# Sudaraka88/LDWeaver

Measured on NVIDIA B200. Metric: weighted SNP-pair MI/sec, higher is better.
Workload: dtype int8 (tcgen05 kind::i8 with int32 accumulation of 28-bit fixed-point weights; fp32 MI epilogue, fp64 refinement of long-range links)

## Files before the change

### ldweaver_b200/csrc/mi_kernel.cuh

```cuda
#pragma once
#include "mi_types.h"
#include "umma.cuh"

namespace ldw {

constexpr int MI_EXP_WARPS = 6;
constexpr int MI_EXP_THREADS = 32 * MI_EXP_WARPS;
constexpr int MI_EPI_WARP0 = 8;
constexpr int MI_EPI_GROUPS = 4;
constexpr int MI_EPI_WARPS = 4 * MI_EPI_GROUPS;
constexpr int MI_EPI_THREADS = 32 * MI_EPI_WARPS;
constexpr int MI_THREADS = 32 * (MI_EPI_WARP0 + MI_EPI_WARPS);
#define LDW_STR2(x) #x
#define LDW_STR(x) LDW_STR2(x)
#define MI_REGS_CTRL 48
#define MI_REGS_EPI 96
static_assert(MI_EPI_WARP0 * 32 * MI_REGS_CTRL + MI_EPI_THREADS * MI_REGS_EPI <= MI_THREADS * ((65536 / MI_THREADS) & ~7), "register budget");
constexpr int MI_MAX_STAGES = 4;
constexpr uint32_t MI_ARR_BYTES = 128 * 128;
constexpr uint32_t MI_STAGE_REGION = 12 * MI_ARR_BYTES;
__host__ __device__ constexpr uint32_t mi_stage_need(int pa, int pb, int njlog2) {
  return (uint32_t)pa * MI_ARR_BYTES + 4u * (uint32_t)pb * (64u << njlog2);
}
__host__ __device__ constexpr int mi_stage_geo(int pa, int pb, int njlog2) {
  return mi_stage_need(pa, pb, njlog2) <= 3 * MI_ARR_BYTES ? 0 : mi_stage_need(pa, pb, njlog2) <= 4 * MI_ARR_BYTES ? 1 : 2;
}
__host__ __device__ constexpr int mi_geo_stages(int geo) { return 4 - geo; }
__host__ __device__ constexpr uint32_t mi_geo_bytes(int geo) { return geo == 0 ? 3 * MI_ARR_BYTES : geo == 1 ? 4 * MI_ARR_BYTES : 6 * MI_ARR_BYTES; }
constexpr uint32_t MI_JREC_BYTES = 128 * sizeof(Rec);
constexpr uint32_t MI_JDYN_BYTES = 128 * sizeof(ColDyn);
constexpr uint32_t MI_IREC_BYTES = 128 * sizeof(Rec);
constexpr uint32_t MI_IDYN_BYTES = 128 * sizeof(RowDyn);
constexpr uint32_t MI_BAR_BYTES = 512;
constexpr uint32_t MI_SMEM_BYTES = MI_STAGE_REGION + 2 * (MI_JREC_BYTES + MI_JDYN_BYTES) + MI_IREC_BYTES + MI_IDYN_BYTES + MI_BAR_BYTES + 1024;
static_assert(MI_SMEM_BYTES <= 232448, "shared memory budget (227 KB opt-in)");

__device__ __forceinline__ float lg2_fast(float x) {
  float y;
  asm("lg2.approx.ftz.f32 %0, %1;" : "=f"(y) : "f"(x));
  return y;
}
__device__ __forceinline__ uint32_t ld_volatile_u32(const uint32_t* p) {
  uint32_t v;
  asm volatile("ld.volatile.global.u32 %0, [%1];" : "=r"(v) : "l"(p));
  return v;
}

__host__ __device__ constexpr int mi_jc(int pa, int pb) {
  return (pa + 1) * (pb + 1) <= 4 ? 8 : (pa + 1) * (pb + 1) <= 9 ? 4 : (pa + 1) * (pb + 1) <= 12 ? 2 : 1;
}
__host__ __device__ constexpr int mi_njlog2(int pa, int pb) {
  return pa * pb == 1 ? 7 : pa * pb == 2 ? 6 : pa * pb <= 4 ? 5 : 4;
}

__device__ __noinline__ void lr_raise_threshold(const ScanParams& p, int lane) {
  constexpr int PER = MI_HIST_BINS / 32;
  uint32_t s = 0;
  for (int k = 0; k < PER; k++) s += ld_volatile_u32(p.hist + lane * PER + k);
  uint32_t suf = s;
#pragma unroll
  for (int o = 1; o < 32; o <<= 1) {
// ... 359 lines not shown
    case 10: epi_tile<3, 3, QC, RG>(p, c, rel); break;
    case 11: epi_tile<3, 4, QC, RG>(p, c, rel); break;
    case 12: epi_tile<4, 1, QC, RG>(p, c, rel); break;
    case 13: epi_tile<4, 2, QC, RG>(p, c, rel); break;
    case 14: epi_tile<4, 3, QC, RG>(p, c, rel); break;
    case 15: epi_tile<4, 4, QC, RG>(p, c, rel); break;
    default: break;
  }
}

template <bool DBG>
__global__ void __cluster_dims__(2, 1, 1) __launch_bounds__(MI_THREADS, 1)
mi_scan_kernel(const __grid_constant__ TmapSet tm, const __grid_constant__ ScanParams p) {
  extern __shared__ uint8_t smem_raw[];
  uint8_t* smem = reinterpret_cast<uint8_t*>((reinterpret_cast<uintptr_t>(smem_raw) + 1023) & ~(uintptr_t)1023);
  uint8_t* stage_base = smem;
  Rec* jrec = reinterpret_cast<Rec*>(smem + MI_STAGE_REGION);
  ColDyn* jdyn = reinterpret_cast<ColDyn*>(smem + MI_STAGE_REGION + 2 * MI_JREC_BYTES);
  Rec* irec = reinterpret_cast<Rec*>(smem + MI_STAGE_REGION + 2 * (MI_JREC_BYTES + MI_JDYN_BYTES));
  RowDyn* idyn = reinterpret_cast<RowDyn*>(smem + MI_STAGE_REGION + 2 * (MI_JREC_BYTES + MI_JDYN_BYTES) + MI_IREC_BYTES);
  uint64_t* bars = reinterpret_cast<uint64_t*>(smem + MI_STAGE_REGION + 2 * (MI_JREC_BYTES + MI_JDYN_BYTES) + MI_IREC_BYTES + MI_IDYN_BYTES);
  uint64_t* full = bars;
  uint64_t* empty = bars + 4;
  uint64_t* ready = bars + 8;
  uint64_t* tfull = bars + 12;
  uint64_t* tempty = bars + 14;
  uint64_t* jfull = bars + 16;
  uint64_t* jempty = bars + 18;
  uint64_t* drained = bars + 20;
  uint64_t* rfull = bars + 21;
  uint64_t* rempty = bars + 22;
  uint32_t* tmem_slot = reinterpret_cast<uint32_t*>(bars + 23);
  uint32_t* thdr = reinterpret_cast<uint32_t*>(bars + 24);

  const int warp = threadIdx.x >> 5, lane = threadIdx.x & 31;
  const uint32_t rank = cluster_ctarank();
  if (warp == 0 && lane == 0) {
    tma_prefetch_desc(&tm.a);
    for (int i = 0; i < MI_MAX_STAGES; i++) {
      mbar_init(&full[i], 1); mbar_init(&empty[i], 1); mbar_init(&ready[i], 2 * MI_EXP_WARPS);
    }
    mbar_init(drained, 1);
    mbar_init(rfull, 1); mbar_init(rempty, MI_EPI_WARPS);
    for (int i = 0; i < 2; i++) {
      mbar_init(&tfull[i], 1); mbar_init(&tempty[i], 2 * MI_EPI_WARPS);
      mbar_init(&jfull[i], 1); mbar_init(&jempty[i], MI_EPI_WARPS);
    }
    fence_barrier_init();
  }
  if (warp == 2) tmem_alloc_pair(tmem_slot, 512);
  tc_fence_before();
  cluster_sync_all();
  tc_fence_after();
  const uint32_t tmem_base = *tmem_slot;
  const int tile0 = (int)(blockIdx.x >> 1), tstep = (int)(gridDim.x >> 1);

  if (warp < MI_EPI_WARP0) {
  asm volatile("setmaxnreg.dec.sync.aligned.u32 " LDW_STR(MI_REGS_CTRL) ";");
  if (warp == 0) {
    int st = 0; uint32_t phb = 0; int geo = -1; uint32_t dph = 0;
    int it = 0, rit = 0;
    long long w_jempty = 0, w_empty = 0, t_begin = DBG ? clock64() : 0;
    for (int t = tile0; t < p.n_tiles; t += tstep, it++) {
      const TileDesc td = p.tiles[t];
      const int PA = td.PA, PB = td.PB, NJ = 1 << td.njlog2, NJh = NJ >> 1;
      const int njidx = 7 - td.njlog2;
      const int g = mi_stage_geo(PA, PB, td.njlog2);
      const int nst = mi_geo_stages(g);
      const uint32_t sbytes = mi_geo_bytes(g);
      if (g != geo) {
        if (geo >= 0) { mbar_wait(drained, dph, 12); dph ^= 1; }
        geo = g; st = 0;
      }
      {
        const uint32_t stage_tx = (uint32_t)PA * MI_ARR_BYTES + (uint32_t)(PB * NJh * 128);
        const int a_row = td.a_row0 + (int)rank * 128, b_row = td.b_row0 + (int)rank * NJh;
        for (int kb = 0; kb < p.nkb; kb++) {
          timed_wait<DBG>(&empty[st], ((phb >> st) & 1) ^ 1, 11, w_empty);
          if (elect_one()) {
            uint8_t* sb = stage_base + st * sbytes;
            mbar_arrive_expect_tx(&full[st], stage_tx);
            for (int a = 0; a < PA; a++)
              tma_load_2d(sb + a * MI_ARR_BYTES, &tm.a, &full[st], kb * 128, a_row + a * td.a_pstride);
            uint8_t* sbB = sb + PA * MI_ARR_BYTES;
            for (int b = 0; b < PB; b++)
              tma_load_2d(sbB + b * NJh * 128, &tm.b[njidx], &full[st], kb * 128, b_row + b * td.b_pstride);
          }
          __syncwarp();
          phb ^= 1u << st;
          if (++st == nst) st = 0;
        }
      }
      const int jb = it & 1;
      timed_wait<DBG>(&jempty[jb], ((it >> 1) & 1) ^ 1, 10, w_jempty);
      if (elect_one()) {
        thdr[jb] = (uint32_t)PA | ((uint32_t)PB << 8) | ((uint32_t)td.njlog2 << 16) | ((uint32_t)(rank ? td.flags1 : td.flags) << 24);
        mbar_arrive_expect_tx(&jfull[jb], (uint32_t)NJ * (uint32_t)(sizeof(Rec) + sizeof(ColDyn)));
        bulk_load_1d(jrec + jb * 128, p.rec + (int64_t)(PA + 1 - 2) * p.rec_vstride + td.j_slot0, NJ * sizeof(Rec), &jfull[jb]);
        bulk_load_1d(jdyn + jb * 128, p.coldyn + td.j_dyn0, NJ * sizeof(ColDyn), &jfull[jb]);
      }
      __syncwarp();
      if (!((rank ? td.flags1 : td.flags) & TILE_NULL)) {
        timed_wait<DBG>(rempty, (uint32_t)(rit & 1) ^ 1, 13, w_jempty);
        if (elect_one()) {
          mbar_arrive_expect_tx(rfull, MI_IREC_BYTES + MI_IDYN_BYTES);
          bulk_load_1d(irec, p.rec + (int64_t)(PB + 1 - 2) * p.rec_vstride + td.i_slot0 + (int)rank * 128, MI_IREC_BYTES, rfull);
          bulk_load_1d(idyn, p.rowdyn + td.i_dyn0 + (int)rank * 128, MI_IDYN_BYTES, rfull);
        }
        __syncwarp();
        rit++;
      }
    }
    if (DBG && p.dbg && lane == 0) {
      p.dbg[blockIdx.x * 16 + 0] = (unsigned long long)(clock64() - t_begin);
      p.dbg[blockIdx.x * 16 + 1] = (unsigned long long)w_jempty;
      p.dbg[blockIdx.x * 16 + 2] = (unsigned long long)w_empty;
    }
  } else if (warp == 1) {
    if (rank == 0) {
    int st = 0; uint32_t phb = 0; int geo = -1; int as = 0; uint32_t aph = 0;
    long long w_tempty = 0, w_ready = 0, t_begin = DBG ? clock64() : 0;
    const uint32_t desc_hi = (uint32_t)(make_smem_desc_sw128(0) >> 32);
    for (int t = tile0; t < p.n_tiles; t += tstep) {
      const TileDesc td = p.tiles[t];
      const int PA = td.PA, PB = td.PB, NJ = 1 << td.njlog2;
      const int g = mi_stage_geo(PA, PB, td.njlog2);
      const int nst = mi_geo_stages(g);
      const uint32_t sbytes = mi_geo_bytes(g);
      if (g != geo) { geo = g; st = 0; }
      bool sw = false;
      if (t + tstep < p.n_tiles) {
        const TileDesc tn = p.tiles[t + tstep];
        sw = mi_stage_geo(tn.PA, tn.PB, tn.njlog2) != g;
      }
      const bool big = 2 * PA * PB * NJ > 256;
      const uint32_t ncols = (uint32_t)(2 * PB * NJ);
      const uint32_t idesc_u = make_idesc_u8(256, ncols);
      const uint32_t idesc_s = make_idesc_s8u8(256, ncols);
      uint32_t dbase;
      if (big) {
        for (int s2 = 0; s2 < 2; s2++) {
          timed_wait<DBG>(&tempty[as], aph ^ 1, 20, w_tempty);
          if (++as == 2) { as = 0; aph ^= 1; }
        }
        dbase = tmem_base;
      } else {
        timed_wait<DBG>(&tempty[as], aph ^ 1, 21, w_tempty);
        dbase = tmem_base + as * 256;
      }
      tc_fence_after();
      {
        const uint32_t boff = (uint32_t)PA * MI_ARR_BYTES;
        const uint32_t b2off = boff + (uint32_t)(PB * NJ * 128);
        for (int kb = 0; kb < p.nkb; kb++) {
          timed_wait<DBG>(&ready[st], (phb >> st) & 1, 22, w_ready);
          tc_fence_after();
          const uint32_t lo = ((smem_u32(stage_base + st * sbytes) & 0x3FFFFu) >> 4) | (1u << 16);
          if (elect_one()) {
            const uint64_t dBa = ((uint64_t)desc_hi << 32) | (lo + (boff >> 4));
            const uint64_t dBb = ((uint64_t)desc_hi << 32) | (lo + (b2off >> 4));
            const uint32_t acc0 = kb > 0 ? 1u : 0u;
            for (int a = 0; a < PA; a++) {
              const uint64_t dx = ((uint64_t)desc_hi << 32) | (lo + (uint32_t)((a * MI_ARR_BYTES) >> 4));
              const uint32_t dHL = dbase + (uint32_t)(a * 2 * PB * NJ);
              umma_i8_pair(dHL, dx, dBa, idesc_u, acc0);
              umma_i8_pair(dHL, dx, dBb, idesc_s, 1u);
#pragma unroll
              for (int kk = 1; kk < 4; kk++) {
                umma_i8_pair(dHL, dx + 2 * kk, dBa + 2 * kk, idesc_u, 1u);
                umma_i8_pair(dHL, dx + 2 * kk, dBb + 2 * kk, idesc_s, 1u);
              }
            }
            umma_commit_pair(&empty[st]);
          }
          __syncwarp();
          phb ^= 1u << st;
          if (++st == nst) st = 0;
        }
      }
      if (elect_one()) {
        if (sw) umma_commit_pair(drained);
        if (big) {
          umma_commit_pair(&tfull[0]);
          umma_commit_pair(&tfull[1]);
        } else {
          umma_commit_pair(&tfull[as]);
        }
      }
      __syncwarp();
      if (!big) {
        if (++as == 2) { as = 0; aph ^= 1; }
      }
    }
    if (DBG && p.dbg && lane == 0) {
      p.dbg[blockIdx.x * 16 + 3] = (unsigned long long)(clock64() - t_begin);
      p.dbg[blockIdx.x * 16 + 4] = (unsigned long long)w_tempty;
      p.dbg[blockIdx.x * 16 + 5] = (unsigned long long)w_ready;
    }
    }
  } else {
    const int h = (warp - 2) * 32 + lane;
    int st = 0; uint32_t phb = 0; int geo = -1;
    long long w_full = 0, t_begin = DBG ? clock64() : 0;
    for (int t = tile0; t < p.n_tiles; t += tstep) {
      const TileDesc td = p.tiles[t];
      const int PA = td.PA, PB = td.PB, NJh = (1 << td.njlog2) >> 1;
      const int brows = PB * NJh;
      const int g = mi_stage_geo(PA, PB, td.njlog2);
      const int nst = mi_geo_stages(g);
      const uint32_t sbytes = mi_geo_bytes(g);
      if (g != geo) { geo = g; st = 0; }
      for (int kb = 0; kb < p.nkb; kb++) {
        const int cl = h & 7;
        const uint8_t* dg = p.dig + (int64_t)kb * 128 + cl * 16;
        const uint4 g0 = __ldg(reinterpret_cast<const uint4*>(dg));
        const uint4 g1 = __ldg(reinterpret_cast<const uint4*>(dg + p.kpad));
        const uint4 g2 = __ldg(reinterpret_cast<const uint4*>(dg + 2 * p.kpad));
        const uint4 g3 = __ldg(reinterpret_cast<const uint4*>(dg + 3 * p.kpad));
        timed_wait<DBG>(&full[st], (phb >> st) & 1, 40, w_full);
        const uint32_t yb = smem_u32(stage_base + st * sbytes) + (uint32_t)PA * MI_ARR_BYTES;
        const uint32_t slot = (uint32_t)brows * 128u;
        for (int r = h >> 3; r < brows; r += MI_EXP_THREADS / 8) {
          const uint32_t addr = yb + (uint32_t)r * 128u + (uint32_t)((cl ^ (r & 7)) * 16);
          const uint4 y = lds128(addr);
          sts128(addr + slot, make_uint4(y.x & g1.x, y.y & g1.y, y.z & g1.z, y.w & g1.w));
          sts128(addr + 2 * slot, make_uint4(y.x & g2.x, y.y & g2.y, y.z & g2.z, y.w & g2.w));
          sts128(addr + 3 * slot, make_uint4(y.x & g3.x, y.y & g3.y, y.z & g3.z, y.w & g3.w));
          sts128(addr, make_uint4(y.x & g0.x, y.y & g0.y, y.z & g0.z, y.w & g0.w));
        }
        fence_proxy_async_smem();
        __syncwarp();
        if (lane == 0) mbar_arrive_cluster(&ready[st], 0);
        phb ^= 1u << st;
        if (++st == nst) st = 0;
      }
    }
    if (DBG && p.dbg && h == 0) {
      p.dbg[blockIdx.x * 16 + 12] = (unsigned long long)(clock64() - t_begin);
      p.dbg[blockIdx.x * 16 + 13] = (unsigned long long)w_full;
    }
  }
  } else {
    asm volatile("setmaxnreg.inc.sync.aligned.u32 " LDW_STR(MI_REGS_EPI) ";");
    EpiCtx c;
    c.q = warp & 3;
    c.cg = (warp - MI_EPI_WARP0) >> 2;
    c.lane = lane;
    c.rank = (int)rank;
    int as = 0; uint32_t aph = 0;
    int it = 0, rit = 0;
    long long w_jfull = 0, w_tfull = 0, t_begin = DBG ? clock64() : 0;
    c.irec_saddr = smem_u32(irec);
    c.idyn_saddr = smem_u32(idyn);
    c.rempty_saddr = smem_u32(rempty);
    c.scr_saddr = smem_u32(bars + 32) + (uint32_t)(warp - MI_EPI_WARP0) * 4u;
    for (int t = tile0; t < p.n_tiles; t += tstep, it++) {
      const int jb = it & 1;
      timed_wait<DBG>(&jfull[jb], (it >> 1) & 1, 30, w_jfull);
      uint32_t hdr;
      asm volatile("ld.shared.u32 %0, [%1];" : "=r"(hdr) : "r"(smem_u32(&thdr[jb])));
      const int tPA = (int)(hdr & 0xFF), tPB = (int)((hdr >> 8) & 0xFF);
      c.tflags = hdr >> 24;
      const int NJ = 1 << ((hdr >> 16) & 0xFF);
      const bool big = 2 * tPA * tPB * NJ > 256;
      if (!(c.tflags & TILE_NULL)) { timed_wait<DBG>(rfull, (uint32_t)(rit & 1), 34, w_jfull); rit++; }
      long long c1 = DBG ? clock64() : 0;
      c.jrec_saddr = smem_u32(jrec + jb * 128);
      c.jdyn_saddr = smem_u32(jdyn + jb * 128);
      if (big) {
        uint32_t ph0 = aph;
        mbar_wait(&tfull[as], ph0, 31);
        int as1 = as ^ 1;
        uint32_t ph1 = (as == 1) ? (aph ^ 1) : aph;
        mbar_wait(&tfull[as1], ph1, 32);
        c.tmem_base = tmem_base + ((uint32_t)(c.q * 32) << 16);
      } else {
        mbar_wait(&tfull[as], aph, 33);
        c.tmem_base = tmem_base + ((uint32_t)(c.q * 32) << 16) + as * 256;
      }
      if constexpr (DBG) w_tfull += clock64() - c1;
      tc_fence_after();
      bool released = false;
      auto release_acc = [&]() {
        tc_fence_before();
        __syncwarp();
        if (big) {
          if (lane == 0) { mbar_arrive_cluster(&tempty[0], 0); mbar_arrive_cluster(&tempty[1], 0); }
          aph ^= 1;
        } else {
// ... 31 lines not shown
```

### ldweaver_b200/csrc/mi_scan.cu

```cuda
#include <algorithm>
#include <chrono>
#include <cmath>
#include <cub/cub.cuh>
#include <vector>

#include "../../include/ldw.h"
#include "ctx.h"
#include "hdw.h"
#include "mi_aux.cuh"
#include "mi_kernel.cuh"
#include "mi_scan.h"

using namespace ldw;

namespace {

struct Group {
  int32_t slot0 = 0, nslots = 0, row0 = 0, count = 0;
};

struct DevLinks {
  DevBuf pos1, pos2, c1, c2, len, blk, mi;
  int ensure(int64_t m) {
    size_t b4 = (size_t)(m > 0 ? m : 1) * 4, b8 = (size_t)(m > 0 ? m : 1) * 8;
// ... 576 lines not shown
  memset(&sp, 0, sizeof(sp));
  sp.tiles = D.tiles.as<TileDesc>();
  sp.n_tiles = H.n_real_tiles;
  sp.rec = P->d_rec.as<Rec>();
  sp.rec_vstride = P->nslots;
  sp.rowdyn = D.rowdyn.as<RowDyn>();
  sp.coldyn = D.coldyn.as<ColDyn>();
  sp.nkb = (int32_t)(P->Kpad / 128);
  sp.nf = H.nf; sp.nt = H.nt;
  sp.diag = H.diag; sp.ragged = H.ragged;
  sp.qcorr = (!H.diag && !(cfg.flags & LDW_SCAN_IDEAL_Q)) ? 1 : 0;
  sp.sr_only = (cfg.flags & LDW_SCAN_SR_ONLY) ? 1 : 0;
  sp.dig = P->d_dig.as<uint8_t>();
  sp.kpad = P->Kpad;
  sp.rfl_arr = D.rfl.as<uint8_t>();
  sp.rtl_arr = D.rtl.as<uint8_t>();
  sp.sa = P->sa;
  sp.sb = P->sb;
  sp.kT = (float)(std::ldexp(1.0, (int)P->sb) / P->scale);
  sp.M = P->M;
  for (int a = 0; a < 4; a++)
    for (int b = 0; b < 4; b++) {
      double ri = a + 2, rj = b + 2;
      double den = P->neff + 0.5 * ri * rj;
      const float den_f = (float)den, rkT = 1.0f / sp.kT, rden = 1.0f / den_f;
      sp.scale[a][b] = (float)(M_LN2 / den) * sp.kT;
      sp.q0s[a][b] = (float)(0.25 * ri * rj / den) * rkT;
      sp.qod[a][b] = (float)(0.25 / den) * rkT;
      sp.rp_qc[a][b] = rden * rkT;
      sp.rp_plain[a][b] = den_f * sp.kT;
    }
}

int launch_scan(const ldw_mi_plan* P, const ScanParams& sp, cudaStream_t st, int reserve = 0) {
  if (sp.n_tiles <= 0) return 0;
  int grid = 2 * std::min<int>(sp.n_tiles, std::max(1, (P->ctx->num_sms - reserve) / 2));
  if (sp.dbg) mi_scan_kernel<true><<<grid, MI_THREADS, MI_SMEM_BYTES, st>>>(P->tm, sp);
  else mi_scan_kernel<false><<<grid, MI_THREADS, MI_SMEM_BYTES, st>>>(P->tm, sp);
  LDW_CUDA(cudaGetLastError());
  return 0;
}

RefineParams make_refine_params(const ldw_mi_plan* P, const BlockDev& D, const BlockHost& H, const ScanCfg& cfg) {
  RefineParams R;
  R.codes = P->codes_dev;
  R.S = P->S;
  R.w = P->d_w.as<double>();
  R.p64 = P->d_p64.as<double>();
  R.r = P->d_r.as<uint8_t>();
  R.mask = P->d_mask.as<uint8_t>();
  R.from_idx = D.from_idx.as<int32_t>();
  R.to_idx = D.to_idx.as<int32_t>();
  R.rfl_arr = D.rfl.as<uint8_t>();
  R.rtl_arr = D.rtl.as<uint8_t>();
  R.nf = H.nf; R.nt = H.nt;
  R.ideal_q = (cfg.flags & LDW_SCAN_IDEAL_Q) ? 1 : 0;
  R.neff = P->neff;
  return R;
}

int validate_scan(const ldw_mi_plan* P, const ScanCfg& cfg) {
  if (!(cfg.g > 0) || cfg.g != std::floor(cfg.g) || cfg.g > 9.0e15) return set_error(LDW_ERR_ARG, "genome length g=%g must be a positive integer", cfg.g);
  if (!(cfg.sr_dist >= 0)) return set_error(LDW_ERR_ARG, "sr_dist must be >= 0");
  if (!P->pos_sorted) return set_error(LDW_ERR_UNSUPPORTED, "POS must be non-decreasing (the short-range slot layout relies on it)");
  if (P->n > 0 && ((double)P->pos.back() - (double)P->pos.front()) >= cfg.g) return set_error(LDW_ERR_UNSUPPORTED, "POS span must be smaller than the genome length g");
  return 0;
}

}
// ... 57 lines not shown
int ldw_mi_block_dense(ldw_mi_plan* P, int64_t block_index, double* mi_out, int64_t* nf_out, int64_t* nt_out) {
  if (!P) return set_error(LDW_ERR_ARG, "null plan");
  LDW_TRY(ctx_bind(P->ctx));
  cudaStream_t st = P->ctx->stream;
  ScanWS* W = get_ws(P->ctx);
  int bf = 0, bt = 0;
  {
    int64_t k = block_index;
    bool found = false;
    for (int i = 0; i < P->nranges && !found; i++)
      for (int j = i; j < P->nranges; j++) {
        if (k == 0) { bf = i; bt = j; found = true; break; }
        k--;
      }
    if (!found) return set_error(LDW_ERR_ARG, "block index out of range");
  }
  ScanCfg cfg{1e15, 0.0, 0, 0, 0};
  cfg.dense = 1;
  BlockHost& H = W->hring[0];
  BlockDev& D = W->ring[0];
  int e = prepare_block(P, bf, bt, cfg, H);
  if (e > 1) return e;
  if (nf_out) *nf_out = H.nf;
  if (nt_out) *nt_out = H.nt;
  if (!mi_out) return 0;
  LDW_TRY(upload_block(st, D, H));
  size_t cells = (size_t)H.nf * H.nt;
  LDW_TRY(W->d_dense.ensure(cells * 4));
  LDW_CUDA(cudaMemsetAsync(W->d_dense.p, 0, cells * 4, st));
  ScanParams sp;
  fill_scan_params(P, D, H, cfg, sp);
  sp.dense = 1;
  sp.dense_out = W->d_dense.as<float>();
  LDW_TRY(launch_scan(P, sp, st));
  DevBuf d64;
  LDW_TRY(d64.alloc(cells * 8));
  f32_to_f64_kernel<<<(unsigned)((cells + 255) / 256), 256, 0, st>>>(W->d_dense.as<float>(), (int64_t)cells, d64.as<double>());
  LDW_CUDA(cudaMemcpyAsync(mi_out, d64.p, cells * 8, cudaMemcpyDeviceToHost, st));
  LDW_CUDA(cudaStreamSynchronize(st));
  return 0;
}

int ldw_mi_pairs_exact(ldw_mi_plan* P, int64_t block_index, const int32_t* from_local, const int32_t* to_local,
                       int64_t n_pairs, double* mi_out) {
  if (!P) return set_error(LDW_ERR_ARG, "null plan");
  LDW_TRY(ctx_bind(P->ctx));
  cudaStream_t st = P->ctx->stream;
  ScanWS* W = get_ws(P->ctx);
  int bf = 0, bt = 0;
  {
    int64_t k = block_index;
    bool found = false;
    for (int i = 0; i < P->nranges && !found; i++)
      for (int j = i; j < P->nranges; j++) {
        if (k == 0) { bf = i; bt = j; found = true; break; }
        k--;
      }
    if (!found) return set_error(LDW_ERR_ARG, "block index out of range");
  }
  if (n_pairs <= 0) return 0;
  ScanCfg cfg{1e15, 0.0, 0, 0, 0};
  BlockHost& H = W->hring[0];
  BlockDev& D = W->ring[0];
  int e = prepare_block(P, bf, bt, cfg, H);
  if (e != 0) return e == 1 ? set_error(LDW_ERR_ARG, "empty block") : e;
  for (int64_t k = 0; k < n_pairs; k++)
    if (from_local[k] < 0 || from_local[k] >= H.nf || to_local[k] < 0 || to_local[k] >= H.nt)
// ... 246 lines not shown
      first_rc = -1;
    } else {
      e = prepare_block(P, blocks[b].bf, blocks[b].bt, cfg, H);
    }
    if (e > 1) return e;
    LDW_TRY(upload_block(P->ctx->upload_stream, D, H));
    LDW_CUDA(cudaEventRecord(D.uploaded, P->ctx->upload_stream));
    LDW_CUDA(cudaStreamWaitEvent(st, D.uploaded, 0));
    host_prep_ms += std::chrono::duration<double, std::milli>(std::chrono::steady_clock::now() - hp0).count();
    D.used = true;
    ScanParams sp;
    fill_scan_params(P, D, H, cfg, sp);
    sp.sr_out = W->d_sr_f32.as<float>() + s.sr_base;
    if (dbg_block >= 0 && (int64_t)b == dbg_block) {
      LDW_TRY(W->d_dbg.ensure(4096 * 16 * 8));
      LDW_CUDA(cudaMemsetAsync(W->d_dbg.p, 0, 4096 * 16 * 8, st));
      sp.dbg = W->d_dbg.as<unsigned long long>();
    }
    const bool lr = !sr_only && s.n_lr > 0;
    const int emit_all = force_emit_all || s.emit_all;
    uint32_t cap = cap_override ? cap_override : s.cap;
    if (lr) {
      if (L.used) LDW_CUDA(cudaStreamWaitEvent(st, L.sel_done, 0));
      const int n_pilot = (int)H.tiles.size() - H.n_real_tiles;
      if (seq == 0 && use_chain && !emit_all && n_pilot > 0) {
        mi_block_begin_kernel<<<1, 256, 0, st>>>(d_count, L.hist.as<uint32_t>(), d_chain, 0);
        ScanParams pp = sp;
        pp.tiles = D.tiles.as<TileDesc>() + H.n_real_tiles;
        pp.n_tiles = n_pilot;
        pp.cand = L.cand.as<Cand>(); pp.cand_cap = cap; pp.cand_count = d_count; pp.tcand_bits = d_tcand;
        pp.hist = L.hist.as<uint32_t>(); pp.kprime = s.kprime; pp.delta = s.delta ? s.delta : 1; pp.overflow = d_overflow;
        pp.emit_all = 1;
        pp.dbg = nullptr;
        LDW_TRY(launch_scan(P, pp, st, 0));
        mi_pilot_seed_kernel<<<1, 1024, 0, st>>>(L.cand.as<Cand>(), d_count, cap, (unsigned long long)s.k_lo, (double)s.n_lr, d_chain);
        LDW_CUDA(cudaGetLastError());
        n_launches += 3;
      }
      if (force_seed >= 0.f && use_chain && !emit_all) {
        static_assert(sizeof(float) == 4, "float bits");
        LDW_CUDA(cudaMemcpyAsync(d_chain, &force_seed, 4, cudaMemcpyHostToDevice, st));
        LDW_CUDA(cudaStreamSynchronize(st));
      }
      mi_block_begin_kernel<<<1, 256, 0, st>>>(d_count, L.hist.as<uint32_t>(), d_chain, (use_chain && !emit_all) ? 1 : 0);
      LDW_CUDA(cudaGetLastError());
      n_launches++;
      sp.cand = L.cand.as<Cand>();
      sp.cand_cap = cap;
      sp.cand_count = d_count;
      sp.tcand_bits = d_tcand;
      sp.hist = L.hist.as<uint32_t>();
      sp.kprime = s.kprime;
      sp.delta = s.delta ? s.delta : 1;
      sp.overflow = d_overflow;
      sp.emit_all = emit_all;
    } else {
      sp.sr_only = 1;
    }
    if (sp.n_tiles > 0) {
      cudaEvent_t k0, k1;
      LDW_CUDA(cudaEventCreate(&k0));
      LDW_CUDA(cudaEventCreate(&k1));
      kev.push_back(k0);
      kev.push_back(k1);
      LDW_CUDA(cudaEventRecord(k0, st));
      LDW_TRY(launch_scan(P, sp, st, lr ? scan_reserve : 0));
      LDW_CUDA(cudaEventRecord(k1, st));
      n_launches++; n_scan_launches++;
      n_tiles += sp.n_tiles;
      for (int32_t ti = 0; ti < H.n_real_tiles; ti++) {
        const TileDesc& td = H.tiles[ti];
        exec_ops += 8.0 * 256.0 * (double)(td.PA * td.PB * (1 << td.njlog2)) * (double)P->Kpad;
        const int RA = td.PA + 1, RB = td.PB + 1;
        const int halves = ((td.flags & TILE_NULL) ? 0 : 1) + ((td.flags1 & TILE_NULL) ? 0 : 1);
        exec_mufu += halves * 128.0 * (double)(1 << td.njlog2) * (double)(RA * (RB + (sp.qcorr ? (RB + 1) / 2 : 0)));
      }
    }
    if (lr) {
      n_launches += 2;
      LDW_CUDA(cudaEventRecord(L.scan_done, st));
      LDW_CUDA(cudaStreamWaitEvent(sst, L.scan_done, 0));
      RefineParams R = make_refine_params(P, D, H, cfg);
      n_launches++;
      mi_presel_kernel<<<1, 1024, 0, sst>>>(L.cand.as<Cand>(), d_count, cap, d_tcand, emit_all, (unsigned long long)s.k_lo, (float)sel_margin,
                                           L.vcand.as<Cand>(), d_count + 5);
      LDW_CUDA(cudaGetLastError());
      mi_refine_list_kernel<<<P->ctx->num_sms * 4, 32 * REFINE_WARPS, 0, sst>>>(R, L.vcand.as<Cand>(), d_count + 5, L.mi64.as<double>());
      LDW_CUDA(cudaGetLastError());
      SelectParams q;
      memset(&q, 0, sizeof(q));
      q.cand = L.vcand.as<Cand>(); q.mi64 = L.mi64.as<double>(); q.vcount = d_count + 5; q.count = d_count; q.cap = cap;
      q.overflow = d_overflow; q.tcand_bits = d_tcand; q.emit_all = emit_all;
      q.k_lo = s.k_lo; q.k_hi = s.k_hi; q.h = s.h; q.interpolate = s.interp;
      q.tol_safe = sel_margin; q.tol_border = 1e-9;
      q.from_idx = D.from_idx.as<int32_t>(); q.to_idx = D.to_idx.as<int32_t>();
      q.nf = H.nf; q.nt = H.nt; q.diag = H.diag; q.block = (int32_t)blocks[b].index;
      q.kept_key = W->d_kept_key.as<uint64_t>(); q.kept_gi = W->d_kept_gi.as<int32_t>(); q.kept_gj = W->d_kept_gj.as<int32_t>();
      q.kept_mi = W->d_kept_mi.as<double>(); q.kept_count = W->d_kept_count.as<unsigned long long>(); q.kept_cap = kept_cap;
      q.kept_overflow = d_kept_overflow;
// ... 226 lines not shown
      double gaps = 0, gmax = 0;
      std::string detail;
      for (size_t k = 1; k + 1 < kev.size(); k += 2) {
        float ms = 0;
        cudaEventElapsedTime(&ms, kev[k], kev[k + 1]);
        gaps += ms;
        gmax = std::max<double>(gmax, ms);
        char b[32];
        snprintf(b, sizeof(b), " %.0f", 1e3 * ms);
        detail += b;
      }
      float first = 0, last = 0;
      cudaEventElapsedTime(&first, ev0, kev[0]);
      cudaEventElapsedTime(&last, kev[kev.size() - 1], ev1);
      fprintf(stderr, "ldw timing: gaps between scan kernels: sum %.3f ms, max %.3f ms; before first %.3f ms, after last %.3f ms; us:%s\n",
              gaps, gmax, first, last, detail.c_str());
    }
    stats_out->n_scan_launches = n_scan_launches;
    stats_out->n_launches = n_launches;
    stats_out->n_tiles = n_tiles;
    stats_out->exec_int8_ops = exec_ops;
    stats_out->t_host_prep_ms = host_prep_ms;
    stats_out->exec_mufu_ops = exec_mufu;
    {
      double em = 0;
      for (size_t b = 0; b < blocks.size(); b++)
        if (!sel[b].skip && sel[b].n_lr > 0 && !sr_only) em = std::max(em, (double)P->results[b].eps_obs);
      stats_out->eps_obs_max = em;
    }
  }
  if (dbg_block >= 0 && W->d_dbg.p) {
    std::vector<unsigned long long> h(4096 * 16);
    cudaMemcpy(h.data(), W->d_dbg.p, h.size() * 8, cudaMemcpyDeviceToHost);
    double s[16] = {0};
    int nb = 0;
    for (int c = 0; c < 4096; c++)
      if (h[c * 16 + 3]) { nb++; for (int k = 0; k < 16; k++) s[k] += (double)h[c * 16 + k]; }
    if (nb) {
      fprintf(stderr, "ldw dbg block %lld (%d CTAs, kilo-cycles avg): producer total %.0f wait_jempty %.0f wait_empty %.0f | "
              "mma total %.0f wait_tempty %.0f wait_ready %.0f | expander total %.0f wait_full %.0f | epi(first) total %.0f "
              "wait_jfull %.0f wait_tfull %.0f | epi(last) total %.0f wait_jfull %.0f wait_tfull %.0f\n", (long long)dbg_block, nb,
              s[0] / nb / 1e3, s[1] / nb / 1e3, s[2] / nb / 1e3, s[3] / nb / 1e3, s[4] / nb / 1e3, s[5] / nb / 1e3, s[12] / nb / 1e3,
              s[13] / nb / 1e3, s[6] / nb / 1e3, s[7] / nb / 1e3, s[8] / nb / 1e3, s[9] / nb / 1e3, s[10] / nb / 1e3, s[11] / nb / 1e3);
    }
  }
  kev_cleanup();
  cudaEventDestroy(ev0); cudaEventDestroy(ev1); cudaEventDestroy(ev2); cudaEventDestroy(ev3);
  lap("borderline + stats (host)");
  return 0;
}
```

### ldweaver_b200/csrc/mi_types.h

```cpp
#pragma once
#include <cuda.h>
#include <stdint.h>

namespace ldw {

struct __align__(16) Rec {
  uint32_t T[4];
  float rp[4];
  float q[4];
  uint32_t T4;
  float rp4;
  float q4;
  uint32_t pad;
};
static_assert(sizeof(Rec) == 64, "Rec must be 64 bytes");

struct RowDyn {
  int32_t il;
  float rtl;
};

struct __align__(16) ColDyn {
  int32_t jl;
  float rfl;
  int32_t a0, a1, b0, b1;
  uint32_t baseU, baseL;
};
static_assert(sizeof(ColDyn) == 32, "ColDyn must be 32 bytes");

enum : uint32_t { TILE_HAS_SR = 1u, TILE_NULL = 2u };

struct __align__(16) TileDesc {
  int32_t a_row0, a_pstride;
  int32_t b_row0, b_pstride;
  int32_t i_slot0, j_slot0;
  int32_t i_dyn0, j_dyn0;
  uint8_t PA, PB, njlog2, flags;
  uint8_t flags1, pad8[3];
  int32_t pad[2];
};
static_assert(sizeof(TileDesc) == 48, "TileDesc must be 48 bytes");

struct Cand {
  int32_t il, jl;
  float mi;
};

constexpr int MI_HIST_BINS = 4096;

struct ScanParams {
  const TileDesc* tiles;
  int32_t n_tiles;
  const Rec* rec;
  int64_t rec_vstride;
  const RowDyn* rowdyn;
  const ColDyn* coldyn;
  int32_t nkb;
  int32_t nf, nt;
  int32_t diag, ragged, qcorr, sr_only, dense, emit_all;
  const uint8_t* rfl_arr;
  const uint8_t* rtl_arr;
  float kT;
  uint32_t sa, sb;
  uint32_t M;
  float scale[4][4];
  float q0s[4][4];
  float qod[4][4];
  float rp_qc[4][4];
  float rp_plain[4][4];
  float* sr_out;
  float* dense_out;
  Cand* cand;
  uint32_t cand_cap;
  uint32_t* cand_count;
  uint32_t* tcand_bits;
  uint32_t* hist;
  uint32_t kprime, delta;
  uint32_t* overflow;
  const uint8_t* dig;
  int64_t kpad;
  unsigned long long* dbg;
};

struct TmapSet {
  CUtensorMap a;
  CUtensorMap b[4];
};

}
```

### ldweaver_b200/csrc/umma.cuh

```cuda
#pragma once
#include <cuda_runtime.h>
#include <stdint.h>
#include <stdio.h>

namespace ldw {

__device__ __forceinline__ uint32_t smem_u32(const void* p) { return (uint32_t)__cvta_generic_to_shared(p); }

__device__ __forceinline__ bool elect_one() {
  uint32_t pred;
  asm volatile(
      "{\n"
      ".reg .pred P;\n"
      "elect.sync _|P, 0xffffffff;\n"
      "selp.u32 %0, 1, 0, P;\n"
      "}\n"
      : "=r"(pred));
  return pred != 0;
}

__device__ __forceinline__ void mbar_init(uint64_t* bar, uint32_t count) {
  asm volatile("mbarrier.init.shared::cta.b64 [%0], %1;" ::"r"(smem_u32(bar)), "r"(count) : "memory");
}
__device__ __forceinline__ void fence_barrier_init() { asm volatile("fence.mbarrier_init.release.cluster;" ::: "memory"); }
__device__ __forceinline__ void fence_proxy_async_smem() { asm volatile("fence.proxy.async.shared::cta;" ::: "memory"); }
__device__ __forceinline__ void mbar_arrive_expect_tx(uint64_t* bar, uint32_t bytes) {
  asm volatile("mbarrier.arrive.expect_tx.shared::cta.b64 _, [%0], %1;" ::"r"(smem_u32(bar)), "r"(bytes) : "memory");
}
__device__ __forceinline__ void mbar_arrive(uint64_t* bar) {
  asm volatile("mbarrier.arrive.shared::cta.b64 _, [%0];" ::"r"(smem_u32(bar)) : "memory");
}
__device__ __forceinline__ bool mbar_try_wait(uint64_t* bar, uint32_t parity) {
  uint32_t ok;
  asm volatile(
      "{\n"
      ".reg .pred p;\n"
      "mbarrier.try_wait.parity.shared::cta.b64 p, [%1], %2, %3;\n"
      "selp.u32 %0, 1, 0, p;\n"
      "}\n"
      : "=r"(ok)
      : "r"(smem_u32(bar)), "r"(parity), "r"(0x989680u)
      : "memory");
  return ok != 0;
}
__device__ __forceinline__ uint64_t globaltimer_ns() {
  uint64_t t;
  asm volatile("mov.u64 %0, %%globaltimer;" : "=l"(t));
  return t;
}
#ifndef LDW_WAIT_TIMEOUT_NS
#define LDW_WAIT_TIMEOUT_NS 4000000000ull
#endif
__device__ __forceinline__ void mbar_wait(uint64_t* bar, uint32_t parity, int tag = 0) {
  if (mbar_try_wait(bar, parity)) return;
  uint32_t spins = 0;
  uint64_t t0 = 0;
  while (!mbar_try_wait(bar, parity)) {
    if ((++spins & 0x3FFu) == 0) {
      uint64_t now = globaltimer_ns();
      if (t0 == 0) t0 = now;
      if (now - t0 > LDW_WAIT_TIMEOUT_NS) {
        printf("ldw: mbarrier wait timeout tag=%d block=%d thread=%d parity=%u\n", tag, (int)blockIdx.x,
               (int)threadIdx.x, parity);
        __trap();
      }
    }
  }
}

__device__ __forceinline__ void mbar_arrive_cluster(uint64_t* bar, uint32_t rank) {
  uint32_t ra;
  asm volatile("mapa.shared::cluster.u32 %0, %1, %2;" : "=r"(ra) : "r"(smem_u32(bar)), "r"(rank));
  asm volatile("mbarrier.arrive.shared::cluster.b64 _, [%0];" ::"r"(ra) : "memory");
}
// ... 146 lines not shown
```

Before: 85.95 billion.

## Keep A rows resident in shared memory across runs of consecutive tiles

Persistent CTAs now process contiguous runs of tiles rather than a strided sequence. When a tile's A panels for all k-blocks fit in shared memory, they stay resident and are reused by following tiles with the same A row, so only B is streamed through a smaller ring; per-slot aempty barriers guard the reuse. The producer also issues the j-record and i-record bulk loads opportunistically inside the k-loop using test_wait, so it no longer blocks on them afterwards. This cuts redundant A TMA traffic, at the cost of fewer B stages, more complex barrier logic, and possible load imbalance from coarser tile runs.

```diff
diff --git a/ldweaver_b200/csrc/mi_kernel.cuh b/ldweaver_b200/csrc/mi_kernel.cuh
--- a/ldweaver_b200/csrc/mi_kernel.cuh
+++ b/ldweaver_b200/csrc/mi_kernel.cuh
@@ -27,6 +27,32 @@
 }
 __host__ __device__ constexpr int mi_geo_stages(int geo) { return 4 - geo; }
 __host__ __device__ constexpr uint32_t mi_geo_bytes(int geo) { return geo == 0 ? 3 * MI_ARR_BYTES : geo == 1 ? 4 * MI_ARR_BYTES : 6 * MI_ARR_BYTES; }
+constexpr int MI_MAX_ASLOTS = (int)(MI_STAGE_REGION / MI_ARR_BYTES);
+__host__ __device__ constexpr uint32_t mi_bstage_bytes(int pb, int njlog2) { return 4u * (uint32_t)pb * (64u << njlog2); }
+__host__ __device__ constexpr int mi_res_stages(int pa, int pb, int njlog2, int nkb) {
+  if (pa * nkb > MI_MAX_ASLOTS) return 0;
+  const uint32_t rest = MI_STAGE_REGION - (uint32_t)(pa * nkb) * MI_ARR_BYTES, b = mi_bstage_bytes(pb, njlog2);
+  return rest >= 4 * b ? 4 : rest >= 3 * b ? 3 : rest >= 2 * b ? 2 : 0;
+}
+struct MiGeo {
+  int id, nst;
+  uint32_t stride, bofs;
+  bool res;
+};
+__host__ __device__ inline MiGeo mi_geo(int pa, int pb, int njlog2, int nkb, bool stream_rows) {
+  const int nr = stream_rows ? 0 : mi_res_stages(pa, pb, njlog2, nkb);
+  MiGeo g;
+  if (nr) {
+    g.stride = mi_bstage_bytes(pb, njlog2);
+    g.id = 0x100 | (pa << 6) | (int)(g.stride >> 10);
+    g.nst = nr; g.bofs = (uint32_t)(pa * nkb) * MI_ARR_BYTES; g.res = true;
+  } else {
+    g.id = mi_stage_geo(pa, pb, njlog2);
+    g.nst = mi_geo_stages(g.id); g.stride = mi_geo_bytes(g.id); g.bofs = (uint32_t)pa * MI_ARR_BYTES; g.res = false;
+  }
+  return g;
+}
+__device__ __forceinline__ int mi_next_tile(int t, int R, int skip) { return (t + 1) % R == 0 ? t + 1 + skip : t + 1; }
 constexpr uint32_t MI_JREC_BYTES = 128 * sizeof(Rec);
 constexpr uint32_t MI_JDYN_BYTES = 128 * sizeof(ColDyn);
 constexpr uint32_t MI_IREC_BYTES = 128 * sizeof(Rec);
@@ -452,6 +478,8 @@
   uint64_t* rempty = bars + 22;
   uint32_t* tmem_slot = reinterpret_cast<uint32_t*>(bars + 23);
   uint32_t* thdr = reinterpret_cast<uint32_t*>(bars + 24);
+  uint64_t* aempty = bars + 40;
+  static_assert((40 + MI_MAX_ASLOTS) * 8 <= MI_BAR_BYTES, "barrier area");
 
   const int warp = threadIdx.x >> 5, lane = threadIdx.x & 31;
   const uint32_t rank = cluster_ctarank();
@@ -460,6 +488,7 @@
     for (int i = 0; i < MI_MAX_STAGES; i++) {
       mbar_init(&full[i], 1); mbar_init(&empty[i], 1); mbar_init(&ready[i], 2 * MI_EXP_WARPS);
     }
+    for (int i = 0; i < MI_MAX_ASLOTS; i++) mbar_init(&aempty[i], 1);
     mbar_init(drained, 1);
     mbar_init(rfull, 1); mbar_init(rempty, MI_EPI_WARPS);
     for (int i = 0; i < 2; i++) {
@@ -473,85 +502,99 @@
   cluster_sync_all();
   tc_fence_after();
   const uint32_t tmem_base = *tmem_slot;
-  const int tile0 = (int)(blockIdx.x >> 1), tstep = (int)(gridDim.x >> 1);
+  const int tile0 = (int)(blockIdx.x >> 1) * p.run_tiles;
+  const int tskip = (int)((gridDim.x >> 1) - 1) * p.run_tiles;
 
   if (warp < MI_EPI_WARP0) {
   asm volatile("setmaxnreg.dec.sync.aligned.u32 " LDW_STR(MI_REGS_CTRL) ";");
   if (warp == 0) {
     int st = 0; uint32_t phb = 0; int geo = -1; uint32_t dph = 0;
     int it = 0, rit = 0;
-    long long w_jempty = 0, w_empty = 0, t_begin = DBG ? clock64() : 0;
-    for (int t = tile0; t < p.n_tiles; t += tstep, it++) {
+    int ra0 = -1, rkind = -1, nrun = 0;
+    long long w_jempty = 0, w_empty = 0, w_aempty = 0, t_begin = DBG ? clock64() : 0;
+    for (int t = tile0; t < p.n_tiles; t = mi_next_tile(t, p.run_tiles, tskip), it++) {
       const TileDesc td = p.tiles[t];
       const int PA = td.PA, PB = td.PB, NJ = 1 << td.njlog2, NJh = NJ >> 1;
       const int njidx = 7 - td.njlog2;
-      const int g = mi_stage_geo(PA, PB, td.njlog2);
-      const int nst = mi_geo_stages(g);
-      const uint32_t sbytes = mi_geo_bytes(g);
-      if (g != geo) {
+      const MiGeo G = mi_geo(PA, PB, td.njlog2, p.nkb, p.stream_rows != 0);
+      if (G.id != geo) {
         if (geo >= 0) { mbar_wait(drained, dph, 12); dph ^= 1; }
-        geo = g; st = 0;
-      }
+        geo = G.id; st = 0;
+      }
+      const bool fresh = !G.res || td.a_row0 != ra0 || (PA | PB << 4) != rkind;
+      ra0 = td.a_row0; rkind = G.res ? (PA | PB << 4) : -1;
+      const int jb = it & 1;
+      bool jdone = false, rdone = ((rank ? td.flags1 : td.flags) & TILE_NULL) != 0;
+      auto load_jrec = [&]() {
+        if (elect_one()) {
+          thdr[jb] = (uint32_t)PA | ((uint32_t)PB << 8) | ((uint32_t)td.njlog2 << 16) | ((uint32_t)(rank ? td.flags1 : td.flags) << 24);
+          mbar_arrive_expect_tx(&jfull[jb], (uint32_t)NJ * (uint32_t)(sizeof(Rec) + sizeof(ColDyn)));
+          bulk_load_1d(jrec + jb * 128, p.rec + (int64_t)(PA + 1 - 2) * p.rec_vstride + td.j_slot0, NJ * sizeof(Rec), &jfull[jb]);
+          bulk_load_1d(jdyn + jb * 128, p.coldyn + td.j_dyn0, NJ * sizeof(ColDyn), &jfull[jb]);
+        }
+        __syncwarp();
+      };
+      auto load_irec = [&]() {
+        if (elect_one()) {
+          mbar_arrive_expect_tx(rfull, MI_IREC_BYTES + MI_IDYN_BYTES);
+          bulk_load_1d(irec, p.rec + (int64_t)(PB + 1 - 2) * p.rec_vstride + td.i_slot0 + (int)rank * 128, MI_IREC_BYTES, rfull);
+          bulk_load_1d(idyn, p.rowdyn + td.i_dyn0 + (int)rank * 128, MI_IDYN_BYTES, rfull);
+        }
+        __syncwarp();
+        rit++;
+      };
       {
-        const uint32_t stage_tx = (uint32_t)PA * MI_ARR_BYTES + (uint32_t)(PB * NJh * 128);
+        const uint32_t stage_tx = (fresh ? (uint32_t)PA * MI_ARR_BYTES : 0u) + (uint32_t)(PB * NJh * 128);
         const int a_row = td.a_row0 + (int)rank * 128, b_row = td.b_row0 + (int)rank * NJh;
         for (int kb = 0; kb < p.nkb; kb++) {
           timed_wait<DBG>(&empty[st], ((phb >> st) & 1) ^ 1, 11, w_empty);
+          if (G.res && fresh && nrun > 0) timed_wait<DBG>(&aempty[kb], (uint32_t)(nrun - 1) & 1, 14, w_aempty);
           if (elect_one()) {
-            uint8_t* sb = stage_base + st * sbytes;
             mbar_arrive_expect_tx(&full[st], stage_tx);
-            for (int a = 0; a < PA; a++)
-              tma_load_2d(sb + a * MI_ARR_BYTES, &tm.a, &full[st], kb * 128, a_row + a * td.a_pstride);
-            uint8_t* sbB = sb + PA * MI_ARR_BYTES;
+            if (fresh) {
+              uint8_t* sa = stage_base + (G.res ? (uint32_t)(kb * PA) * MI_ARR_BYTES : st * G.stride);
+              for (int a = 0; a < PA; a++)
+                tma_load_2d(sa + a * MI_ARR_BYTES, &tm.a, &full[st], kb * 128, a_row + a * td.a_pstride);
+            }
+            uint8_t* sbB = stage_base + G.bofs + st * G.stride;
             for (int b = 0; b < PB; b++)
               tma_load_2d(sbB + b * NJh * 128, &tm.b[njidx], &full[st], kb * 128, b_row + b * td.b_pstride);
           }
           __syncwarp();
           phb ^= 1u << st;
-          if (++st == nst) st = 0;
-        }
-      }
-      const int jb = it & 1;
-      timed_wait<DBG>(&jempty[jb], ((it >> 1) & 1) ^ 1, 10, w_jempty);
-      if (elect_one()) {
-        thdr[jb] = (uint32_t)PA | ((uint32_t)PB << 8) | ((uint32_t)td.njlog2 << 16) | ((uint32_t)(rank ? td.flags1 : td.flags) << 24);
-        mbar_arrive_expect_tx(&jfull[jb], (uint32_t)NJ * (uint32_t)(sizeof(Rec) + sizeof(ColDyn)));
-        bulk_load_1d(jrec + jb * 128, p.rec + (int64_t)(PA + 1 - 2) * p.rec_vstride + td.j_slot0, NJ * sizeof(Rec), &jfull[jb]);
-        bulk_load_1d(jdyn + jb * 128, p.coldyn + td.j_dyn0, NJ * sizeof(ColDyn), &jfull[jb]);
-      }
-      __syncwarp();
-      if (!((rank ? td.flags1 : td.flags) & TILE_NULL)) {
-        timed_wait<DBG>(rempty, (uint32_t)(rit & 1) ^ 1, 13, w_jempty);
-        if (elect_one()) {
-          mbar_arrive_expect_tx(rfull, MI_IREC_BYTES + MI_IDYN_BYTES);
-          bulk_load_1d(irec, p.rec + (int64_t)(PB + 1 - 2) * p.rec_vstride + td.i_slot0 + (int)rank * 128, MI_IREC_BYTES, rfull);
-          bulk_load_1d(idyn, p.rowdyn + td.i_dyn0 + (int)rank * 128, MI_IDYN_BYTES, rfull);
-        }
-        __syncwarp();
-        rit++;
-      }
+          if (++st == G.nst) st = 0;
+          if (!jdone && __shfl_sync(0xffffffffu, (int)mbar_test_wait(&jempty[jb], ((it >> 1) & 1) ^ 1), 0)) { load_jrec(); jdone = true; }
+          if (jdone && !rdone && __shfl_sync(0xffffffffu, (int)mbar_test_wait(rempty, (uint32_t)(rit & 1) ^ 1), 0)) { load_irec(); rdone = true; }
+        }
+        if (G.res && fresh) nrun++;
+      }
+      if (!jdone) { timed_wait<DBG>(&jempty[jb], ((it >> 1) & 1) ^ 1, 10, w_jempty); load_jrec(); }
+      if (!rdone) { timed_wait<DBG>(rempty, (uint32_t)(rit & 1) ^ 1, 13, w_jempty); load_irec(); }
     }
     if (DBG && p.dbg && lane == 0) {
       p.dbg[blockIdx.x * 16 + 0] = (unsigned long long)(clock64() - t_begin);
       p.dbg[blockIdx.x * 16 + 1] = (unsigned long long)w_jempty;
       p.dbg[blockIdx.x * 16 + 2] = (unsigned long long)w_empty;
+      p.dbg[blockIdx.x * 16 + 14] = (unsigned long long)w_aempty;
     }
   } else if (warp == 1) {
     if (rank == 0) {
     int st = 0; uint32_t phb = 0; int geo = -1; int as = 0; uint32_t aph = 0;
     long long w_tempty = 0, w_ready = 0, t_begin = DBG ? clock64() : 0;
     const uint32_t desc_hi = (uint32_t)(make_smem_desc_sw128(0) >> 32);
-    for (int t = tile0; t < p.n_tiles; t += tstep) {
+    for (int t = tile0; t < p.n_tiles; t = mi_next_tile(t, p.run_tiles, tskip)) {
       const TileDesc td = p.tiles[t];
       const int PA = td.PA, PB = td.PB, NJ = 1 << td.njlog2;
-      const int g = mi_stage_geo(PA, PB, td.njlog2);
-      const int nst = mi_geo_stages(g);
-      const uint32_t sbytes = mi_geo_bytes(g);
-      if (g != geo) { geo = g; st = 0; }
-      bool sw = false;
-      if (t + tstep < p.n_tiles) {
-        const TileDesc tn = p.tiles[t + tstep];
-        sw = mi_stage_geo(tn.PA, tn.PB, tn.njlog2) != g;
+      const MiGeo G = mi_geo(PA, PB, td.njlog2, p.nkb, p.stream_rows != 0);
+      if (G.id != geo) { geo = G.id; st = 0; }
+      bool sw = false, last = G.res;
+      {
+        const int tn = mi_next_tile(t, p.run_tiles, tskip);
+        if (tn < p.n_tiles) {
+          const TileDesc dn = p.tiles[tn];
+          sw = mi_geo(dn.PA, dn.PB, dn.njlog2, p.nkb, p.stream_rows != 0).id != G.id;
+          last = G.res && (dn.a_row0 != td.a_row0 || dn.PA != PA || dn.PB != PB);
+        }
       }
       const bool big = 2 * PA * PB * NJ > 256;
       const uint32_t ncols = (uint32_t)(2 * PB * NJ);
@@ -570,18 +613,18 @@
       }
       tc_fence_after();
       {
-        const uint32_t boff = (uint32_t)PA * MI_ARR_BYTES;
-        const uint32_t b2off = boff + (uint32_t)(PB * NJ * 128);
+        const uint32_t b2off = (uint32_t)(PB * NJ * 128);
         for (int kb = 0; kb < p.nkb; kb++) {
           timed_wait<DBG>(&ready[st], (phb >> st) & 1, 22, w_ready);
           tc_fence_after();
-          const uint32_t lo = ((smem_u32(stage_base + st * sbytes) & 0x3FFFFu) >> 4) | (1u << 16);
+          const uint32_t alo = ((smem_u32(stage_base + (G.res ? (uint32_t)(kb * PA) * MI_ARR_BYTES : st * G.stride)) & 0x3FFFFu) >> 4) | (1u << 16);
+          const uint32_t blo = ((smem_u32(stage_base + G.bofs + st * G.stride) & 0x3FFFFu) >> 4) | (1u << 16);
           if (elect_one()) {
-            const uint64_t dBa = ((uint64_t)desc_hi << 32) | (lo + (boff >> 4));
-            const uint64_t dBb = ((uint64_t)desc_hi << 32) | (lo + (b2off >> 4));
+            const uint64_t dBa = ((uint64_t)desc_hi << 32) | blo;
+            const uint64_t dBb = ((uint64_t)desc_hi << 32) | (blo + (b2off >> 4));
             const uint32_t acc0 = kb > 0 ? 1u : 0u;
             for (int a = 0; a < PA; a++) {
-              const uint64_t dx = ((uint64_t)desc_hi << 32) | (lo + (uint32_t)((a * MI_ARR_BYTES) >> 4));
+              const uint64_t dx = ((uint64_t)desc_hi << 32) | (alo + (uint32_t)((a * MI_ARR_BYTES) >> 4));
               const uint32_t dHL = dbase + (uint32_t)(a * 2 * PB * NJ);
               umma_i8_pair(dHL, dx, dBa, idesc_u, acc0);
               umma_i8_pair(dHL, dx, dBb, idesc_s, 1u);
@@ -592,10 +635,11 @@
               }
             }
             umma_commit_pair(&empty[st]);
+            if (last) umma_commit_pair(&aempty[kb]);
           }
           __syncwarp();
           phb ^= 1u << st;
-          if (++st == nst) st = 0;
+          if (++st == G.nst) st = 0;
         }
       }
       if (elect_one()) {
@@ -622,14 +666,12 @@
     const int h = (warp - 2) * 32 + lane;
     int st = 0; uint32_t phb = 0; int geo = -1;
     long long w_full = 0, t_begin = DBG ? clock64() : 0;
-    for (int t = tile0; t < p.n_tiles; t += tstep) {
+    for (int t = tile0; t < p.n_tiles; t = mi_next_tile(t, p.run_tiles, tskip)) {
       const TileDesc td = p.tiles[t];
       const int PA = td.PA, PB = td.PB, NJh = (1 << td.njlog2) >> 1;
       const int brows = PB * NJh;
-      const int g = mi_stage_geo(PA, PB, td.njlog2);
-      const int nst = mi_geo_stages(g);
-      const uint32_t sbytes = mi_geo_bytes(g);
-      if (g != geo) { geo = g; st = 0; }
+      const MiGeo G = mi_geo(PA, PB, td.njlog2, p.nkb, p.stream_rows != 0);
+      if (G.id != geo) { geo = G.id; st = 0; }
       for (int kb = 0; kb < p.nkb; kb++) {
         const int cl = h & 7;
         const uint8_t* dg = p.dig + (int64_t)kb * 128 + cl * 16;
@@ -638,7 +680,7 @@
         const uint4 g2 = __ldg(reinterpret_cast<const uint4*>(dg + 2 * p.kpad));
         const uint4 g3 = __ldg(reinterpret_cast<const uint4*>(dg + 3 * p.kpad));
         timed_wait<DBG>(&full[st], (phb >> st) & 1, 40, w_full);
-        const uint32_t yb = smem_u32(stage_base + st * sbytes) + (uint32_t)PA * MI_ARR_BYTES;
+        const uint32_t yb = smem_u32(stage_base + G.bofs + st * G.stride);
         const uint32_t slot = (uint32_t)brows * 128u;
         for (int r = h >> 3; r < brows; r += MI_EXP_THREADS / 8) {
           const uint32_t addr = yb + (uint32_t)r * 128u + (uint32_t)((cl ^ (r & 7)) * 16);
@@ -652,7 +694,7 @@
         __syncwarp();
         if (lane == 0) mbar_arrive_cluster(&ready[st], 0);
         phb ^= 1u << st;
-        if (++st == nst) st = 0;
+        if (++st == G.nst) st = 0;
       }
     }
     if (DBG && p.dbg && h == 0) {
@@ -674,7 +716,7 @@
     c.idyn_saddr = smem_u32(idyn);
     c.rempty_saddr = smem_u32(rempty);
     c.scr_saddr = smem_u32(bars + 32) + (uint32_t)(warp - MI_EPI_WARP0) * 4u;
-    for (int t = tile0; t < p.n_tiles; t += tstep, it++) {
+    for (int t = tile0; t < p.n_tiles; t = mi_next_tile(t, p.run_tiles, tskip), it++) {
       const int jb = it & 1;
       timed_wait<DBG>(&jfull[jb], (it >> 1) & 1, 30, w_jfull);
       uint32_t hdr;
diff --git a/ldweaver_b200/csrc/mi_scan.cu b/ldweaver_b200/csrc/mi_scan.cu
--- a/ldweaver_b200/csrc/mi_scan.cu
+++ b/ldweaver_b200/csrc/mi_scan.cu
@@ -632,9 +632,32 @@
     }
 }
 
-int launch_scan(const ldw_mi_plan* P, const ScanParams& sp, cudaStream_t st, int reserve = 0) {
-  if (sp.n_tiles <= 0) return 0;
-  int grid = 2 * std::min<int>(sp.n_tiles, std::max(1, (P->ctx->num_sms - reserve) / 2));
+static_assert(mi_res_stages(1, 1, 7, 5) == 3 && mi_res_stages(2, 2, 5, 5) == 2 && mi_res_stages(2, 4, 4, 5) == 2 &&
+              mi_res_stages(1, 3, 5, 5) == 4 && mi_res_stages(3, 1, 5, 5) == 0 && mi_res_stages(1, 1, 7, 16) == 0,
+              "resident-row geometry");
+
+constexpr int MI_RUN_MAX = 16;
+int pick_run_tiles(const TileDesc* tiles, int n, int npairs, int nkb, bool stream_rows) {
+  bool res = false;
+  for (int i = 0; i < n && !res && !stream_rows; i++) res = mi_res_stages(tiles[i].PA, tiles[i].PB, tiles[i].njlog2, nkb) > 0;
+  if (!res || n <= npairs) return 1;
+  const int q = (n + npairs - 1) / npairs, lim = q + std::max(1, q / 100);
+  for (int R = MI_RUN_MAX; R > 1; R--) {
+    const int round = npairs * R, most = (n / round) * R + std::min(R, n % round);
+    if (most <= lim) return R;
+  }
+  return 1;
+}
+
+int launch_scan(const ldw_mi_plan* P, const ScanParams& sp0, const TileDesc* htiles, cudaStream_t st, int reserve = 0) {
+  if (sp0.n_tiles <= 0) return 0;
+  ScanParams sp = sp0;
+  const int npairs = std::min<int>(sp.n_tiles, std::max(1, (P->ctx->num_sms - reserve) / 2));
+  const int grid = 2 * npairs;
+  const char* e = getenv("LDW_DBG_STREAM_ROWS");
+  sp.stream_rows = (e && atoi(e) != 0) ? 1 : 0;
+  sp.run_tiles = pick_run_tiles(htiles, sp.n_tiles, npairs, sp.nkb, sp.stream_rows != 0);
+  if (const char* r = getenv("LDW_DBG_RUN_TILES")) sp.run_tiles = std::max(1, std::min(atoi(r), (int)sp.n_tiles));
   if (sp.dbg) mi_scan_kernel<true><<<grid, MI_THREADS, MI_SMEM_BYTES, st>>>(P->tm, sp);
   else mi_scan_kernel<false><<<grid, MI_THREADS, MI_SMEM_BYTES, st>>>(P->tm, sp);
   LDW_CUDA(cudaGetLastError());
@@ -758,7 +781,7 @@
   fill_scan_params(P, D, H, cfg, sp);
   sp.dense = 1;
   sp.dense_out = W->d_dense.as<float>();
-  LDW_TRY(launch_scan(P, sp, st));
+  LDW_TRY(launch_scan(P, sp, H.tiles.data(), st));
   DevBuf d64;
   LDW_TRY(d64.alloc(cells * 8));
   f32_to_f64_kernel<<<(unsigned)((cells + 255) / 256), 256, 0, st>>>(W->d_dense.as<float>(), (int64_t)cells, d64.as<double>());
@@ -1071,7 +1094,7 @@
         pp.hist = L.hist.as<uint32_t>(); pp.kprime = s.kprime; pp.delta = s.delta ? s.delta : 1; pp.overflow = d_overflow;
         pp.emit_all = 1;
         pp.dbg = nullptr;
-        LDW_TRY(launch_scan(P, pp, st, 0));
+        LDW_TRY(launch_scan(P, pp, H.tiles.data() + H.n_real_tiles, st, 0));
         mi_pilot_seed_kernel<<<1, 1024, 0, st>>>(L.cand.as<Cand>(), d_count, cap, (unsigned long long)s.k_lo, (double)s.n_lr, d_chain);
         LDW_CUDA(cudaGetLastError());
         n_launches += 3;
@@ -1103,7 +1126,7 @@
       kev.push_back(k0);
       kev.push_back(k1);
       LDW_CUDA(cudaEventRecord(k0, st));
-      LDW_TRY(launch_scan(P, sp, st, lr ? scan_reserve : 0));
+      LDW_TRY(launch_scan(P, sp, H.tiles.data(), st, lr ? scan_reserve : 0));
       LDW_CUDA(cudaEventRecord(k1, st));
       n_launches++; n_scan_launches++;
       n_tiles += sp.n_tiles;
@@ -1396,16 +1419,21 @@
   if (dbg_block >= 0 && W->d_dbg.p) {
     std::vector<unsigned long long> h(4096 * 16);
     cudaMemcpy(h.data(), W->d_dbg.p, h.size() * 8, cudaMemcpyDeviceToHost);
-    double s[16] = {0};
+    double s[16] = {0}, tmin = 1e300, tmax = 0;
     int nb = 0;
     for (int c = 0; c < 4096; c++)
-      if (h[c * 16 + 3]) { nb++; for (int k = 0; k < 16; k++) s[k] += (double)h[c * 16 + k]; }
+      if (h[c * 16 + 3]) {
+        nb++;
+        for (int k = 0; k < 16; k++) s[k] += (double)h[c * 16 + k];
+        tmin = std::min(tmin, (double)h[c * 16 + 6]); tmax = std::max(tmax, (double)h[c * 16 + 6]);
+      }
     if (nb) {
-      fprintf(stderr, "ldw dbg block %lld (%d CTAs, kilo-cycles avg): producer total %.0f wait_jempty %.0f wait_empty %.0f | "
-              "mma total %.0f wait_tempty %.0f wait_ready %.0f | expander total %.0f wait_full %.0f | epi(first) total %.0f "
-              "wait_jfull %.0f wait_tfull %.0f | epi(last) total %.0f wait_jfull %.0f wait_tfull %.0f\n", (long long)dbg_block, nb,
-              s[0] / nb / 1e3, s[1] / nb / 1e3, s[2] / nb / 1e3, s[3] / nb / 1e3, s[4] / nb / 1e3, s[5] / nb / 1e3, s[12] / nb / 1e3,
-              s[13] / nb / 1e3, s[6] / nb / 1e3, s[7] / nb / 1e3, s[8] / nb / 1e3, s[9] / nb / 1e3, s[10] / nb / 1e3, s[11] / nb / 1e3);
+      fprintf(stderr, "ldw dbg block %lld (%d CTAs, kilo-cycles avg): producer total %.0f wait_jempty %.0f wait_empty %.0f "
+              "wait_aempty %.0f | mma total %.0f wait_tempty %.0f wait_ready %.0f | expander total %.0f wait_full %.0f | epi(first) total %.0f "
+              "wait_jfull %.0f wait_tfull %.0f | epi(last) total %.0f wait_jfull %.0f wait_tfull %.0f | finish min %.0f max %.0f\n",
+              (long long)dbg_block, nb, s[0] / nb / 1e3, s[1] / nb / 1e3, s[2] / nb / 1e3, s[14] / nb / 1e3, s[3] / nb / 1e3,
+              s[4] / nb / 1e3, s[5] / nb / 1e3, s[12] / nb / 1e3, s[13] / nb / 1e3, s[6] / nb / 1e3, s[7] / nb / 1e3,
+              s[8] / nb / 1e3, s[9] / nb / 1e3, s[10] / nb / 1e3, s[11] / nb / 1e3, tmin / 1e3, tmax / 1e3);
     }
   }
   kev_cleanup();
diff --git a/ldweaver_b200/csrc/mi_types.h b/ldweaver_b200/csrc/mi_types.h
--- a/ldweaver_b200/csrc/mi_types.h
+++ b/ldweaver_b200/csrc/mi_types.h
@@ -56,6 +56,8 @@
   const RowDyn* rowdyn;
   const ColDyn* coldyn;
   int32_t nkb;
+  int32_t run_tiles;
+  int32_t stream_rows;
   int32_t nf, nt;
   int32_t diag, ragged, qcorr, sr_only, dense, emit_all;
   const uint8_t* rfl_arr;
diff --git a/ldweaver_b200/csrc/umma.cuh b/ldweaver_b200/csrc/umma.cuh
--- a/ldweaver_b200/csrc/umma.cuh
+++ b/ldweaver_b200/csrc/umma.cuh
@@ -40,6 +40,19 @@
       "}\n"
       : "=r"(ok)
       : "r"(smem_u32(bar)), "r"(parity), "r"(0x989680u)
+      : "memory");
+  return ok != 0;
+}
+__device__ __forceinline__ bool mbar_test_wait(uint64_t* bar, uint32_t parity) {
+  uint32_t ok;
+  asm volatile(
+      "{\n"
+      ".reg .pred p;\n"
+      "mbarrier.test_wait.parity.shared::cta.b64 p, [%1], %2;\n"
+      "selp.u32 %0, 1, 0, p;\n"
+      "}\n"
+      : "=r"(ok)
+      : "r"(smem_u32(bar)), "r"(parity)
       : "memory");
   return ok != 0;
 }
```

Result: slower. 69.31 billion (median of 6 runs) (-19.4%).
